# harshad16/odh-kubeflow

Measured on AMD Instinct MI355X. Metric: Notebook-CR reconciles/sec + p50 pod-Ready latency at 1/2/4/8 GPU pods, higher is better.
Workload: dtype n/a

## Files before the change

odh_kubeflow_amd/native/objcore.cpp:

```cpp
#define PY_SSIZE_T_CLEAN
#include <Python.h>

#include <cerrno>
#include <cmath>
#include <cstdio>
#include <cstdlib>
#include <cstring>
#include <string>
#include <string_view>
#include <unordered_map>
#include <utility>
#include <vector>

namespace {

PyObject* copy_tree(PyObject* o, int depth) {
  if (depth > 512) {
    PyErr_SetString(PyExc_RecursionError, "object tree too deep");
    return nullptr;
  }
  if (PyDict_CheckExact(o)) {
    PyObject* out = _PyDict_NewPresized(PyDict_GET_SIZE(o));
    if (!out) return nullptr;
    Py_ssize_t pos = 0;
    PyObject *k, *v;
    while (PyDict_Next(o, &pos, &k, &v)) {
      PyObject* c = copy_tree(v, depth + 1);
// ... 742 lines not shown
PyObject* py_loads_shared(PyObject*, PyObject* args) {
  PyObject *data, *old = Py_None;
  if (!PyArg_ParseTuple(args, "O|O", &data, &old)) return nullptr;
  Parser ps;
  if (!init_parser(data, &ps)) return nullptr;
  PyObject* out = value(ps, old == Py_None ? nullptr : old, 0);
  if (!out) return nullptr;
  ws(ps);
  if (ps.p != ps.end) {
    Py_DECREF(out);
    return fail(ps, "extra data");
  }
  return out;
}

PyObject* py_loads_event(PyObject*, PyObject* args) {
  PyObject *data, *lookup = Py_None;
  if (!PyArg_ParseTuple(args, "O|O", &data, &lookup)) return nullptr;
  Parser ps;
  if (!init_parser(data, &ps)) return nullptr;
  ws(ps);
  if (ps.p >= ps.end || *ps.p != '{') return fail(ps, "an event is an object");
  ++ps.p;
  PyObject* type = nullptr;
  PyObject* obj = nullptr;
  PyObject* ret = nullptr;
  ws(ps);
  if (ps.p < ps.end && *ps.p == '}') {
    ++ps.p;
  } else {
    while (true) {
      ws(ps);
      if (ps.p >= ps.end || *ps.p != '"') {
        fail(ps, "expected a key");
        goto done;
// ... 53 lines not shown
  }
  ws(ps);
  if (ps.p != ps.end) {
    fail(ps, "extra data");
    goto done;
  }
  if (!obj) obj = PyDict_New();
  if (!obj) goto done;
  ret = PyTuple_Pack(2, type ? type : Py_None, obj);
done:
  Py_XDECREF(type);
  Py_XDECREF(obj);
  return ret;
}


bool enc_value(std::string& out, PyObject* o, int depth);

void enc_string(std::string& out, PyObject* u) {
  Py_ssize_t n;
  const char* s = PyUnicode_AsUTF8AndSize(u, &n);
  out.push_back('"');
  const char* run = s;
  for (Py_ssize_t i = 0; i < n; ++i) {
    unsigned char c = static_cast<unsigned char>(s[i]);
    if (c >= 0x20 && c != '"' && c != '\\') continue;
    out.append(run, static_cast<size_t>(s + i - run));
    run = s + i + 1;
    switch (c) {
      case '"': out.append("\\\""); break;
// ... 100 lines not shown
  }
  PyErr_SetString(PyExc_TypeError, "not a JSON tree");
  return false;
}

PyObject* py_dumps(PyObject*, PyObject* o) {
  std::string out;
  out.reserve(1024);
  if (!enc_value(out, o, 0)) {
    if (!PyErr_Occurred()) PyErr_SetString(PyExc_TypeError, "not a JSON tree");
    return nullptr;
  }
  return PyBytes_FromStringAndSize(out.data(), static_cast<Py_ssize_t>(out.size()));
}

PyMethodDef methods[] = {
    {"dumps", py_dumps, METH_O,
     "dumps(obj) -> bytes: compact JSON (json.dumps with separators=(',', ':'), UTF-8) of a JSON tree."},
    {"deepcopy", py_deepcopy, METH_O, "Deep copy of a JSON tree (dict/list; tuples become lists)."},
    {"semantic_equal", py_semantic_equal, METH_VARARGS,
     "Structural equality treating missing/None/{}/[] map values as equal."},
    {"equal_except", py_equal_except, METH_VARARGS, "a == b ignoring the given metadata keys."},
    {"loads_shared", py_loads_shared, METH_VARARGS,
     "loads_shared(data, old=None): json.loads, reusing the subtrees of old the document leaves unchanged."},
    {"loads_event", py_loads_event, METH_VARARGS,
     "loads_event(line, lookup=None) -> (type, object): a watch event, the object decoded against "
     "lookup(namespace, name)."},
    {nullptr, nullptr, 0, nullptr}};

PyModuleDef module = {PyModuleDef_HEAD_INIT, "_objcore", "Native JSON-tree core", -1, methods,
                      nullptr, nullptr, nullptr, nullptr};

}

PyMODINIT_FUNC PyInit__objcore(void) {
  if (!g_keys) g_keys = new std::unordered_map<std::string_view, PyObject*>();
  return PyModule_Create(&module);
}
```

odh_kubeflow_amd/ops/build.py:

```python

from __future__ import annotations

import os
import shutil
import subprocess
import sys
import sysconfig
from typing import Dict, List

HERE = os.path.dirname(os.path.abspath(__file__))
CSRC = os.path.join(HERE, "csrc")
LIBDIR = os.path.join(HERE, "_lib")
NATIVE = os.path.join(os.path.dirname(HERE), "native")
TEST_NATIVE = os.path.join(os.path.dirname(HERE), "testing", "native")
OBJCORE = "_objcore" + (sysconfig.get_config_var("EXT_SUFFIX") or ".so")
ARCH = os.environ.get("ODH_GPU_ARCH", "gfx950")
ROCM = os.environ.get("ROCM_PATH", "/opt/rocm")
PROBE_EXE = "odh-gpu-probe"


def _hipcc() -> str:
    p = os.path.join(ROCM, "bin", "hipcc")
    return p if os.path.exists(p) else (shutil.which("hipcc") or p)

# ... 3 lines not shown
        "libodh_gpu_probe.so": {
            "src": [os.path.join(CSRC, "gpu_probe.hip"), os.path.join(CSRC, "probe_cli.cpp")],
            "deps": [os.path.join(CSRC, "gpu_probe.h"), os.path.join(CSRC, "gpu_probe_mx.h"),
                     os.path.join(CSRC, "gpu_probe_dense.h")],
            "cmd": lambda src, out: [_hipcc(), f"--offload-arch={ARCH}", "-O3", "-std=c++17", "-shared", "-fPIC",
                                     *src, "-o", out],
        },
        PROBE_EXE: {
            "src": [os.path.join(CSRC, "probe_main.cpp")],
            "deps": [os.path.join(LIBDIR, "libodh_gpu_probe.so")],
            "cmd": lambda src, out: [_hipcc(), "-O2", "-std=c++17", *src, f"-L{LIBDIR}", "-lodh_gpu_probe",
                                     "-Wl,-rpath,$ORIGIN", "-o", out],
        },
        OBJCORE: {
            "src": [os.path.join(NATIVE, "objcore.cpp")],
            "out": os.path.join(NATIVE, OBJCORE),
            "cmd": lambda src, out: [os.environ.get("CXX", "g++"), "-O2", "-std=c++17", "-shared", "-fPIC", "-Wall",
                                     "-fno-strict-aliasing", f"-I{sysconfig.get_paths()['include']}", *src,
                                     "-o", out],
        },
        "odh-apiserver": {
            "src": [os.path.join(TEST_NATIVE, "apiserver", "apiserver.cpp")],
            "deps": [os.path.join(TEST_NATIVE, "apiserver", "json.hpp")],
            "out": os.path.join(TEST_NATIVE, "bin", "odh-apiserver"),
            "cmd": lambda src, out: [os.environ.get("CXX", "g++"), "-O2", "-std=c++17", "-pthread", "-Wall", *src,
                                     "-o", out, "-lssl", "-lcrypto"],
        },
        "libodh_gpu_telemetry.so": {
            "src": [os.path.join(CSRC, "gpu_telemetry.cpp")],
            "cmd": lambda src, out: [os.environ.get("CXX", "g++"), "-O2", "-std=c++17", "-shared", "-fPIC",
# ... 47 lines not shown
```

odh_kubeflow_amd/runtime/http1.py:

```python

from __future__ import annotations

import asyncio
import os
import ssl as _ssl
import sys
import time
from typing import AsyncIterator, Dict, List, Optional, Tuple
from urllib.parse import urlsplit


class HttpError(Exception):
    pass


def _parse_head(raw: bytes) -> Tuple[int, Dict[str, str]]:
    lines = raw.decode("latin-1").split("\r\n")
    parts = lines[0].split(" ", 2)
    if len(parts) < 2 or not parts[0].startswith("HTTP/"):
        raise HttpError(f"bad status line {lines[0]!r}")
    headers = {}
    for line in lines[1:]:
        if ":" in line:
            k, v = line.split(":", 1)
# ... 41 lines not shown
    _LAG_LOOPS.add(id(loop))

    async def watch() -> None:
        while True:
            t0 = time.perf_counter()
            await asyncio.sleep(0.002)
            late = (time.perf_counter() - t0 - 0.002) * 1e3
            if late >= _STALL_MS:
                _stall_report(f"event loop {late:.1f} ms late")

    loop.create_task(watch())


class _Conn(asyncio.Protocol):

    def __init__(self):
        self.transport = None
        self.buf = bytearray()
        self.closed = False
        self._waiter: Optional[asyncio.Future] = None
        self._head: Optional[Tuple[int, Dict[str, str]]] = None
        self._body = bytearray()
        self._want = -1
        self._streaming = False
        self._lines: List[bytes] = []
        self._got = 0
        self._eof = False
        self._no_body = False


    def connection_made(self, transport) -> None:
        self.transport = transport

    def data_received(self, data: bytes) -> None:
        self.buf += data
        if self._waiter is not None or self._streaming:
            self._advance()

    def eof_received(self):
        return False

    def connection_lost(self, exc) -> None:
        self.closed = True
        self._eof = True
        w, self._waiter = self._waiter, None
        if w is None or w.done():
            return
        if self._streaming:
            w.set_result(None)
        elif self._want == -3 and self._head is not None:
            self._body += self.buf
            self.buf.clear()
            w.set_result((self._head[0], bytes(self._body), True))
        else:
            w.set_exception(ConnectionResetError(f"connection lost mid-response: {exc!r}"))


    def _advance(self) -> None:
        w = self._waiter
        try:
            if self._head is None:
                i = self.buf.find(b"\r\n\r\n")
                if i < 0:
                    return
                self._head = _parse_head(bytes(self.buf[:i]))
                del self.buf[:i + 4]
                status, h = self._head
                if self._no_body or status < 200 or status in (204, 304):
                    self._want = 0
                elif h.get("transfer-encoding", "").lower() == "chunked":
# ... 54 lines not shown
            del body[:start]
        if done:
            self._eof = True
            self.close()
        w = self._waiter
        if (self._lines or self._eof) and w is not None and not w.done():
            self._waiter = None
            w.set_result(None)


    async def roundtrip(self, payload: bytes) -> Tuple[int, bytes, bool]:
        if self.closed:
            raise ConnectionResetError("connection closed")
        self._waiter = w = asyncio.get_running_loop().create_future()
        self._no_body = payload.startswith(b"HEAD ")
        self.transport.write(payload)
        if self.buf:
            self._advance()
        return await w

    async def open_stream(self, payload: bytes) -> Tuple[int, Dict[str, str]]:
        if self.closed:
            raise ConnectionResetError("connection closed")
        self._streaming = True
        self._waiter = w = asyncio.get_running_loop().create_future()
        self.transport.write(payload)
        got = await w
        if got is None:
            raise ConnectionResetError("connection lost before the response head")
        return got

    async def next_lines(self) -> List[bytes]:
        while not self._lines:
            if self._eof or self.closed:
                return []
            self._waiter = w = asyncio.get_running_loop().create_future()
            try:
                await w
            finally:
                if self._waiter is w:
                    self._waiter = None
        out, self._lines = self._lines, []
        return out

    def close(self) -> None:
        self.closed = True
        if self.transport is not None:
            self.transport.close()


class Http1Pool:
    def __init__(self, base_url: str, ssl_context: Optional[_ssl.SSLContext] = None,
                 headers: Optional[Dict[str, str]] = None, size: int = 64, spare: int = 0):
        u = urlsplit(base_url)
        self.host = u.hostname or "127.0.0.1"
        self.port = u.port or (443 if u.scheme == "https" else 80)
        self.ssl = ssl_context if u.scheme == "https" else None
        self._hdr = {"Host": f"{self.host}:{self.port}", "Accept": "application/json"}
        self._hdr.update(headers or {})
        self._static = "".join(f"{k}: {v}\r\n" for k, v in self._hdr.items())
        self._idle: List[_Conn] = []
        self.size = size
        self.opened = 0
        self.spare = max(0, int(spare))
        self._warming = 0

    def set_header(self, name: str, value: Optional[str]) -> None:
        if value is None:
            self._hdr.pop(name, None)
        else:
            self._hdr[name] = value
        self._static = "".join(f"{k}: {v}\r\n" for k, v in self._hdr.items())

    async def _connect(self) -> _Conn:
        loop = asyncio.get_running_loop()
        transport, conn = await loop.create_connection(_Conn, self.host, self.port, ssl=self.ssl)
        sock = transport.get_extra_info("socket")
        if sock is not None:
            import socket

            try:
                sock.setsockopt(socket.IPPROTO_TCP, socket.TCP_NODELAY, 1)
            except OSError:
                pass
        self.opened += 1
        return conn

    def _head(self, method: str, target: str, body: Optional[bytes], content_type: Optional[str]) -> bytes:
        h = f"{method} {target} HTTP/1.1\r\n{self._static}"
        if body is not None:
            h += f"Content-Type: {content_type or 'application/json'}\r\nContent-Length: {len(body)}\r\n"
# ... 66 lines not shown
            raise
        return status, headers, _Stream(conn)

    async def close(self) -> None:
        self.spare = 0
        for c in self._idle:
            c.close()
        self._idle.clear()


class _Stream:

    def __init__(self, conn: _Conn):
        self.conn = conn

    async def read_all(self) -> bytes:
        try:
            out = []
            while True:
                got = await self.conn.next_lines()
                if not got:
                    break
                out += [x + b"\n" for x in got]
            return b"".join(out) + bytes(self.conn._body)
        finally:
            self.close()

    async def batches(self) -> AsyncIterator[List[bytes]]:
        try:
            while True:
                got = await self.conn.next_lines()
                if not got:
                    return
                yield got
        finally:
            self.close()

    async def lines(self) -> AsyncIterator[bytes]:
        async for batch in self.batches():
            for line in batch:
                yield line

    def close(self) -> None:
        self.conn.close()



_REASONS = {200: "OK", 400: "Bad Request", 404: "Not Found", 405: "Method Not Allowed", 413: "Payload Too Large",
            500: "Internal Server Error"}
Handler = "Callable[[str, str, Dict[str, str], bytes], Awaitable[Tuple[int, str, bytes]]]"


class Http1Server:

    def __init__(self, handler, host: str = "127.0.0.1", port: int = 0,
                 ssl_context: Optional[_ssl.SSLContext] = None, max_body: int = 16 << 20, reuse_port: bool = False,
                 max_requests_per_conn: int = 0):
        self.handler = handler
        self.reuse_port = reuse_port
        self.max_requests_per_conn = max_requests_per_conn
        self.host = host
        self.port = port
        self.ssl = ssl_context
        self.max_body = max_body
        self._server = None
        self._conns: set = set()

    async def start(self) -> "Http1Server":
        if _STALL_MS:
            _ensure_loop_watchdog()
        self._server = await asyncio.start_server(self._serve, self.host, self.port, ssl=self.ssl, limit=1 << 24,
                                                  reuse_port=self.reuse_port or None)
        self.port = self._server.sockets[0].getsockname()[1]
        return self

    async def _serve(self, reader, writer) -> None:
        task = asyncio.current_task()
        self._conns.add(task)
        sock = writer.get_extra_info("socket")
        if sock is not None:
            import socket

            try:
                sock.setsockopt(socket.IPPROTO_TCP, socket.TCP_NODELAY, 1)
            except OSError:
                pass
        served = 0
        try:
            while True:
                try:
                    raw = await reader.readuntil(b"\r\n\r\n")
                except (asyncio.IncompleteReadError, ConnectionError, OSError, _ssl.SSLError):
                    return
                lines = raw.decode("latin-1").split("\r\n")
                parts = lines[0].split(" ")
                if len(parts) < 3:
                    return
                method, target = parts[0], parts[1]
                headers = {}
                for line in lines[1:]:
                    if ":" in line:
                        k, v = line.split(":", 1)
                        headers[k.strip().lower()] = v.strip()
                n = int(headers.get("content-length", "0") or 0)
                if n > self.max_body:
                    status, ctype, body = 413, "text/plain", b"request body too large"
                else:
                    data = await reader.readexactly(n) if n else b""
                    try:
                        status, ctype, body = await self.handler(method, target.split("?", 1)[0], headers, data)
                    except Exception as e:
                        status, ctype, body = 500, "text/plain", repr(e).encode()
                served += 1
                close = headers.get("connection", "").lower() == "close" or (
                    self.max_requests_per_conn > 0 and served >= self.max_requests_per_conn)
                head = (f"HTTP/1.1 {status} {_REASONS.get(status, 'OK')}\r\nContent-Type: {ctype}\r\n"
                        f"Content-Length: {len(body)}\r\n{'Connection: close' + chr(13) + chr(10) if close else ''}\r\n")
                writer.write(head.encode("latin-1") + body)
                await writer.drain()
                if close:
                    return
        except (ConnectionError, OSError, asyncio.IncompleteReadError):
            return
        finally:
            self._conns.discard(task)
            try:
                writer.close()
            except Exception:
                pass

    async def stop(self) -> None:
        if self._server is not None:
            self._server.close()
            for t in list(self._conns):
                t.cancel()
            try:
                await asyncio.wait_for(self._server.wait_closed(), 2.0)
            except (asyncio.TimeoutError, Exception):
                pass
            self._server = None
```

odh_kubeflow_amd/runtime/rest.py:

```python

from __future__ import annotations

import asyncio
import base64
import json
import logging
import os
import ssl
import tempfile
import time
from dataclasses import dataclass, field
from typing import Any, AsyncIterator, Dict, List, Optional, Tuple

try:
    from ..native._objcore import dumps as _dumps
    from ..native._objcore import loads_event as _loads_event
    from ..native._objcore import loads_shared as _loads_shared

    def loads_json(raw):
        try:
            return _loads_shared(raw)
        except ValueError:
            return json.loads(raw)

# ... 165 lines not shown
            self.t = now
            if self.tokens >= 1:
                self.tokens -= 1
                return
            await asyncio.sleep((1 - self.tokens) / self.qps)


def _info_and_version(ref) -> Tuple[ResourceInfo, str]:
    info = SCHEME.resolve(ref)
    return info, _version_of(ref) or info.storage_version


class RestClient(Client):
    GET_RETRIES = 10

    def __init__(self, config: RestConfig, pool: int = 64):
        self.config = config
        self.base = config.host.rstrip("/")
        self._ssl = config.ssl_context()
        self._session = None
        self._pool = pool
        self._bucket = TokenBucket(config.qps, config.burst)
        self.requests = 0
        self.by_verb: Dict[str, int] = {}
        self.bytes_in: Dict[str, int] = {}
        from collections import deque

        self.get_ms = deque(maxlen=8192)
        self.retries = 0
        self.user = config.user_agent
        self._discovery: dict = {}
        self.tokens: Optional[FileTokenSource] = (FileTokenSource(config.token_file, config.token)
                                                  if config.token_file else None)
        self._sent_token: Optional[str] = None
        self.token_retries = 0

    def _bearer(self) -> Optional[str]:
        return self.tokens.token() if self.tokens is not None else self.config.token

    def _http(self):
        from .http1 import Http1Pool

        tok = self._bearer()
        if self._session is None:
            headers = {"User-Agent": self.config.user_agent}
            if tok:
                headers["Authorization"] = f"Bearer {tok}"
            self._session = Http1Pool(self.base, self._ssl, headers, size=self._pool, spare=2)
            self._sent_token = tok
        elif tok != self._sent_token:
            self._session.set_header("Authorization", f"Bearer {tok}" if tok else None)
            self._sent_token = tok
        return self._session

    def _unauthorized_retry(self, status: int, sent: Optional[str]) -> bool:
        if status != 401 or self.tokens is None:
            return False
        self.tokens.refresh()
        if self.tokens.token() == sent:
            return False
        self.token_retries += 1
        return True

# ... 190 lines not shown
            if self._unauthorized_retry(status, sent):
                status, _headers, stream = await self._http().stream("GET", target)
            else:
                status, _headers, stream = 401, _headers, None
        if stream is None:
            raise ApiError.from_status({"code": 401, "reason": "Unauthorized", "message": "Unauthorized"}, 401)
        if status >= 400:
            raw = await stream.read_all()
            try:
                raise ApiError.from_status(json.loads(raw), status)
            except ValueError:
                raise InternalError(raw[:200].decode(errors="replace"))
        loads = json.loads
        native = _loads_event
        try:
            async for lines in stream.batches():
                out = []
                err = None
                for line in lines:
                    if not line or line.isspace():
                        continue
                    if native is not None:
                        try:
                            et, obj = native(line, lookup)
                        except ValueError:
                            ev = loads(line)
                            et, obj = ev.get("type"), ev.get("object") or {}
                    else:
                        ev = loads(line)
                        et, obj = ev.get("type"), ev.get("object") or {}
# ... 13 lines not shown
```

Before: 3396.

## Move HTTP/1.1 framing and watch-stream decoding into native C++ parser

Adds a C++ wire framer (wire.hpp) exposed as ResponseParser, WatchDecoder and RequestParser types in _objcore. The client pool, the test server and the watch loop use them to frame responses, de-chunk watch bodies, split lines and decode events in one native call, replacing per-line Python work. The server switches from asyncio streams to a Protocol backed by the native request parser. The aim is lower Python overhead per request and per watch event, at the cost of a large new native parsing surface with its own edge cases and error handling.

```diff
diff --git a/odh_kubeflow_amd/native/objcore.cpp b/odh_kubeflow_amd/native/objcore.cpp
--- a/odh_kubeflow_amd/native/objcore.cpp
+++ b/odh_kubeflow_amd/native/objcore.cpp
@@ -6,11 +6,14 @@
 #include <cstdio>
 #include <cstdlib>
 #include <cstring>
+#include <new>
 #include <string>
 #include <string_view>
 #include <unordered_map>
 #include <utility>
 #include <vector>
+
+#include "wire.hpp"
 
 namespace {
 
@@ -783,11 +786,7 @@
   return out;
 }
 
-PyObject* py_loads_event(PyObject*, PyObject* args) {
-  PyObject *data, *lookup = Py_None;
-  if (!PyArg_ParseTuple(args, "O|O", &data, &lookup)) return nullptr;
-  Parser ps;
-  if (!init_parser(data, &ps)) return nullptr;
+PyObject* decode_event(Parser& ps, PyObject* lookup) {
   ws(ps);
   if (ps.p >= ps.end || *ps.p != '{') return fail(ps, "an event is an object");
   ++ps.p;
@@ -871,6 +870,14 @@
   return ret;
 }
 
+PyObject* py_loads_event(PyObject*, PyObject* args) {
+  PyObject *data, *lookup = Py_None;
+  if (!PyArg_ParseTuple(args, "O|O", &data, &lookup)) return nullptr;
+  Parser ps;
+  if (!init_parser(data, &ps)) return nullptr;
+  return decode_event(ps, lookup);
+}
+
 
 bool enc_value(std::string& out, PyObject* o, int depth);
 
@@ -1001,6 +1008,364 @@
   return PyBytes_FromStringAndSize(out.data(), static_cast<Py_ssize_t>(out.size()));
 }
 
+
+PyObject* wire_error(const std::string& what) {
+  PyErr_Format(PyExc_ValueError, "malformed HTTP message: %s", what.empty() ? "?" : what.c_str());
+  return nullptr;
+}
+
+inline PyObject* view_bytes(wire::View v) {
+  return PyBytes_FromStringAndSize(v.p, static_cast<Py_ssize_t>(v.n));
+}
+
+inline PyObject* view_latin1(wire::View v) {
+  return PyUnicode_DecodeLatin1(v.p ? v.p : "", static_cast<Py_ssize_t>(v.n), nullptr);
+}
+
+bool append_owned(PyObject* list, PyObject* item) {
+  if (!item) return false;
+  int rc = PyList_Append(list, item);
+  Py_DECREF(item);
+  return rc == 0;
+}
+
+struct ResponseParserObj {
+  PyObject_HEAD
+  wire::ResponseFramer* f;
+};
+
+PyObject* rp_new(PyTypeObject* t, PyObject*, PyObject*) {
+  auto* self = reinterpret_cast<ResponseParserObj*>(t->tp_alloc(t, 0));
+  if (!self) return nullptr;
+  self->f = new (std::nothrow) wire::ResponseFramer();
+  if (!self->f) {
+    Py_DECREF(self);
+    return PyErr_NoMemory();
+  }
+  return reinterpret_cast<PyObject*>(self);
+}
+
+void rp_dealloc(PyObject* o) {
+  delete reinterpret_cast<ResponseParserObj*>(o)->f;
+  Py_TYPE(o)->tp_free(o);
+}
+
+PyObject* response_tuple(const wire::Response& r) {
+  PyObject* body = view_bytes(r.body);
+  if (!body) return nullptr;
+  PyObject* t = Py_BuildValue("(iNO)", r.status, body, r.close ? Py_True : Py_False);
+  return t;
+}
+
+PyObject* rp_feed(PyObject* o, PyObject* arg) {
+  auto* self = reinterpret_cast<ResponseParserObj*>(o);
+  Py_buffer b;
+  if (PyObject_GetBuffer(arg, &b, PyBUF_SIMPLE) < 0) return nullptr;
+  PyObject* out = PyList_New(0);
+  const char* p = static_cast<const char*>(b.buf);
+  size_t n = static_cast<size_t>(b.len);
+  try {
+    while (out) {
+      size_t used = 0;
+      wire::Response r;
+      wire::Result got = self->f->next(p, n, &used, &r);
+      if (got == wire::kError) {
+        Py_CLEAR(out);
+        wire_error(self->f->error());
+        break;
+      }
+      if (got == wire::kNeedMore) break;
+      if (!append_owned(out, response_tuple(r))) Py_CLEAR(out);
+      p += used;
+      n -= used;
+      if (n == 0 && !self->f->mid_response()) break;
+    }
+  } catch (...) {
+    Py_CLEAR(out);
+    PyErr_NoMemory();
+  }
+  PyBuffer_Release(&b);
+  return out;
+}
+
+PyObject* rp_finish(PyObject* o, PyObject*) {
+  auto* self = reinterpret_cast<ResponseParserObj*>(o);
+  wire::Response r;
+  if (self->f->finish(&r) == wire::kReady) return response_tuple(r);
+  Py_RETURN_NONE;
+}
+
+PyObject* rp_set_head(PyObject* o, PyObject* arg) {
+  int v = PyObject_IsTrue(arg);
+  if (v < 0) return nullptr;
+  reinterpret_cast<ResponseParserObj*>(o)->f->set_head_request(v != 0);
+  Py_RETURN_NONE;
+}
+
+PyObject* rp_feed_head(PyObject* o, PyObject* arg) {
+  auto* self = reinterpret_cast<ResponseParserObj*>(o);
+  Py_buffer b;
+  if (PyObject_GetBuffer(arg, &b, PyBUF_SIMPLE) < 0) return nullptr;
+  PyObject* out = nullptr;
+  try {
+    size_t used = 0;
+    wire::ResponseHead h;
+    wire::BodyMode mode;
+    uint64_t length;
+    wire::Result got = self->f->head(static_cast<const char*>(b.buf), static_cast<size_t>(b.len), &used, &h, &mode,
+                                     &length);
+    if (got == wire::kError) {
+      wire_error(self->f->error());
+    } else if (got == wire::kNeedMore) {
+      out = Py_None;
+      Py_INCREF(out);
+    } else {
+      out = Py_BuildValue("(iOiKy#)", h.status, h.close ? Py_True : Py_False, static_cast<int>(mode),
+                          static_cast<unsigned long long>(length), static_cast<const char*>(b.buf) + used,
+                          static_cast<Py_ssize_t>(static_cast<size_t>(b.len) - used));
+    }
+  } catch (...) {
+    PyErr_NoMemory();
+  }
+  PyBuffer_Release(&b);
+  return out;
+}
+
+PyMethodDef rp_methods[] = {
+    {"feed", rp_feed, METH_O, "feed(data) -> [(status, body, close), ...]"},
+    {"finish", rp_finish, METH_NOARGS, "finish() -> (status, body, True) or None: the connection ended"},
+    {"set_head", rp_set_head, METH_O, "set_head(flag): the next response answers a HEAD"},
+    {"feed_head", rp_feed_head, METH_O, "feed_head(data) -> None or (status, close, mode, length, rest)"},
+    {nullptr, nullptr, 0, nullptr}};
+
+PyTypeObject ResponseParserType{};
+
+struct WatchDecoderObj {
+  PyObject_HEAD
+  wire::StreamFramer* f;
+  bool busy;
+};
+
+PyObject* wd_new(PyTypeObject* t, PyObject* args, PyObject*) {
+  int mode = wire::kChunked;
+  unsigned long long length = 0;
+  if (!PyArg_ParseTuple(args, "|iK", &mode, &length)) return nullptr;
+  if (mode < wire::kLength || mode > wire::kUntilEof) {
+    PyErr_SetString(PyExc_ValueError, "mode is 0 (length), 1 (chunked) or 2 (until EOF)");
+    return nullptr;
+  }
+  auto* self = reinterpret_cast<WatchDecoderObj*>(t->tp_alloc(t, 0));
+  if (!self) return nullptr;
+  self->busy = false;
+  self->f = new (std::nothrow) wire::StreamFramer(static_cast<wire::BodyMode>(mode), length);
+  if (!self->f) {
+    Py_DECREF(self);
+    return PyErr_NoMemory();
+  }
+  return reinterpret_cast<PyObject*>(self);
+}
+
+void wd_dealloc(PyObject* o) {
+  delete reinterpret_cast<WatchDecoderObj*>(o)->f;
+  Py_TYPE(o)->tp_free(o);
+}
+
+inline bool blank_line(const char* p, size_t n) {
+  for (size_t i = 0; i < n; ++i) {
+    char c = p[i];
+    if (!(c == ' ' || (c >= '\t' && c <= '\r'))) return false;
+  }
+  return true;
+}
+
+PyObject* wd_run(WatchDecoderObj* self, PyObject* data, PyObject* lookup, bool decode) {
+  if (self->busy) {
+    PyErr_SetString(PyExc_RuntimeError, "WatchDecoder.feed re-entered from its lookup");
+    return nullptr;
+  }
+  Py_buffer b;
+  if (PyObject_GetBuffer(data, &b, PyBUF_SIMPLE) < 0) return nullptr;
+  PyObject* out = PyList_New(0);
+  bool ok = out != nullptr;
+  wire::Result got = wire::kNeedMore;
+  self->busy = true;
+  try {
+    Parser ps;
+    auto line = [&](const char* p, size_t n) {
+      if (!ok) return;
+      if (!decode) {
+        ok = append_owned(out, PyBytes_FromStringAndSize(p, static_cast<Py_ssize_t>(n)));
+        return;
+      }
+      if (blank_line(p, n)) return;
+      ps.p = p;
+      ps.end = p + n;
+      PyObject* ev = decode_event(ps, lookup);
+      if (!ev && PyErr_ExceptionMatches(PyExc_ValueError)) {
+        PyErr_Clear();
+        ev = PyBytes_FromStringAndSize(p, static_cast<Py_ssize_t>(n));
+      }
+      ok = append_owned(out, ev);
+    };
+    if (ok) got = self->f->feed(static_cast<const char*>(b.buf), static_cast<size_t>(b.len), line);
+  } catch (...) {
+    if (ok) PyErr_NoMemory();
+    ok = false;
+  }
+  self->busy = false;
+  PyBuffer_Release(&b);
+  if (ok && got == wire::kError) {
+    ok = false;
+    wire_error("bad chunk");
+  }
+  if (!ok) {
+    Py_XDECREF(out);
+    return nullptr;
+  }
+  return Py_BuildValue("(NO)", out, got == wire::kReady ? Py_True : Py_False);
+}
+
+PyObject* wd_feed(PyObject* o, PyObject* args) {
+  PyObject *data, *lookup = Py_None;
+  if (!PyArg_ParseTuple(args, "O|O", &data, &lookup)) return nullptr;
+  return wd_run(reinterpret_cast<WatchDecoderObj*>(o), data, lookup, true);
+}
+
+PyObject* wd_feed_lines(PyObject* o, PyObject* data) {
+  return wd_run(reinterpret_cast<WatchDecoderObj*>(o), data, Py_None, false);
+}
+
+PyObject* wd_rest(PyObject* o, PyObject*) {
+  const std::string& r = reinterpret_cast<WatchDecoderObj*>(o)->f->rest();
+  return PyBytes_FromStringAndSize(r.data(), static_cast<Py_ssize_t>(r.size()));
+}
+
+PyObject* wd_done(PyObject* o, PyObject*) {
+  return PyBool_FromLong(reinterpret_cast<WatchDecoderObj*>(o)->f->done());
+}
+
+PyMethodDef wd_methods[] = {
+    {"feed", wd_feed, METH_VARARGS, "feed(data, lookup=None) -> (events, done)"},
+    {"feed_lines", wd_feed_lines, METH_O, "feed_lines(data) -> (lines, done)"},
+    {"rest", wd_rest, METH_NOARGS, "rest() -> bytes after the last newline"},
+    {"done", wd_done, METH_NOARGS, "done() -> the body has ended"},
+    {nullptr, nullptr, 0, nullptr}};
+
+PyTypeObject WatchDecoderType{};
+
+struct RequestParserObj {
+  PyObject_HEAD
+  wire::RequestFramer* f;
+};
+
+PyObject* rq_new(PyTypeObject* t, PyObject* args, PyObject*) {
+  unsigned long long max_body = 16ull << 20;
+  if (!PyArg_ParseTuple(args, "|K", &max_body)) return nullptr;
+  auto* self = reinterpret_cast<RequestParserObj*>(t->tp_alloc(t, 0));
+  if (!self) return nullptr;
+  self->f = new (std::nothrow) wire::RequestFramer(max_body);
+  if (!self->f) {
+    Py_DECREF(self);
+    return PyErr_NoMemory();
+  }
+  return reinterpret_cast<PyObject*>(self);
+}
+
+void rq_dealloc(PyObject* o) {
+  delete reinterpret_cast<RequestParserObj*>(o)->f;
+  Py_TYPE(o)->tp_free(o);
+}
+
+PyObject* request_tuple(const wire::Request& r) {
+  PyObject* headers = PyDict_New();
+  if (!headers) return nullptr;
+  for (const auto& kv : r.headers) {
+    PyObject* k = view_latin1(kv.first);
+    PyObject* v = view_latin1(kv.second);
+    int rc = (k && v) ? PyDict_SetItem(headers, k, v) : -1;
+    Py_XDECREF(k);
+    Py_XDECREF(v);
+    if (rc < 0) {
+      Py_DECREF(headers);
+      return nullptr;
+    }
+  }
+  PyObject* body;
+  if (r.too_large) {
+    body = Py_None;
+    Py_INCREF(body);
+  } else {
+    body = view_bytes(r.body);
+  }
+  PyObject* method = view_latin1(r.method);
+  PyObject* path = view_latin1(r.path);
+  if (!body || !method || !path) {
+    Py_XDECREF(body);
+    Py_XDECREF(method);
+    Py_XDECREF(path);
+    Py_DECREF(headers);
+    return nullptr;
+  }
+  return Py_BuildValue("(NNNN)", method, path, headers, body);
+}
+
+PyObject* rq_feed(PyObject* o, PyObject* arg) {
+  auto* self = reinterpret_cast<RequestParserObj*>(o);
+  Py_buffer b;
+  if (PyObject_GetBuffer(arg, &b, PyBUF_SIMPLE) < 0) return nullptr;
+  PyObject* out = PyList_New(0);
+  const char* p = static_cast<const char*>(b.buf);
+  size_t n = static_cast<size_t>(b.len);
+  try {
+    wire::Request r;
+    while (out) {
+      size_t used = 0;
+      wire::Result got = self->f->next(p, n, &used, &r);
+      if (got == wire::kError) {
+        Py_CLEAR(out);
+        wire_error(self->f->error());
+        break;
+      }
+      if (got == wire::kNeedMore) break;
+      if (!append_owned(out, request_tuple(r))) Py_CLEAR(out);
+      p += used;
+      n -= used;
+      if (n == 0) break;
+    }
+  } catch (...) {
+    Py_CLEAR(out);
+    PyErr_NoMemory();
+  }
+  PyBuffer_Release(&b);
+  return out;
+}
+
+PyMethodDef rq_methods[] = {
+    {"feed", rq_feed, METH_O, "feed(data) -> [(method, path, headers, body), ...]"},
+    {nullptr, nullptr, 0, nullptr}};
+
+PyTypeObject RequestParserType{};
+
+bool add_type(PyObject* m, PyTypeObject* t, const char* name, const char* qualname, size_t size, newfunc nw,
+              destructor de, PyMethodDef* meths, const char* doc) {
+  PyObject* as_object = reinterpret_cast<PyObject*>(t);
+  if (Py_REFCNT(as_object) == 0) Py_SET_REFCNT(as_object, 1);
+  t->tp_name = qualname;
+  t->tp_basicsize = static_cast<Py_ssize_t>(size);
+  t->tp_flags = Py_TPFLAGS_DEFAULT;
+  t->tp_new = nw;
+  t->tp_dealloc = de;
+  t->tp_methods = meths;
+  t->tp_doc = doc;
+  if (PyType_Ready(t) < 0) return false;
+  Py_INCREF(t);
+  if (PyModule_AddObject(m, name, reinterpret_cast<PyObject*>(t)) < 0) {
+    Py_DECREF(t);
+    return false;
+  }
+  return true;
+}
+
 PyMethodDef methods[] = {
     {"dumps", py_dumps, METH_O,
      "dumps(obj) -> bytes: compact JSON (json.dumps with separators=(',', ':'), UTF-8) of a JSON tree."},
@@ -1022,5 +1387,17 @@
 
 PyMODINIT_FUNC PyInit__objcore(void) {
   if (!g_keys) g_keys = new std::unordered_map<std::string_view, PyObject*>();
-  return PyModule_Create(&module);
-}
+  PyObject* m = PyModule_Create(&module);
+  if (!m) return nullptr;
+  if (!add_type(m, &ResponseParserType, "ResponseParser", "_objcore.ResponseParser", sizeof(ResponseParserObj), rp_new,
+                rp_dealloc, rp_methods, "Incremental HTTP/1.1 response framing (client side).") ||
+      !add_type(m, &WatchDecoderType, "WatchDecoder", "_objcore.WatchDecoder", sizeof(WatchDecoderObj), wd_new,
+                wd_dealloc, wd_methods,
+                "WatchDecoder(mode=1, length=0): a streaming body framed, split into lines and decoded.") ||
+      !add_type(m, &RequestParserType, "RequestParser", "_objcore.RequestParser", sizeof(RequestParserObj), rq_new,
+                rq_dealloc, rq_methods, "RequestParser(max_body=16 MiB): incremental HTTP/1.1 request framing.")) {
+    Py_DECREF(m);
+    return nullptr;
+  }
+  return m;
+}
diff --git a/odh_kubeflow_amd/native/wire.hpp b/odh_kubeflow_amd/native/wire.hpp
--- /dev/null
+++ b/odh_kubeflow_amd/native/wire.hpp
@@ -0,0 +1,570 @@
+#pragma once
+
+#include <cstddef>
+#include <cstdint>
+#include <cstring>
+#include <string>
+#include <utility>
+#include <vector>
+
+namespace wire {
+
+enum Result { kNeedMore = 0, kReady = 1, kError = -1 };
+enum BodyMode { kLength = 0, kChunked = 1, kUntilEof = 2 };
+
+constexpr size_t kMaxHead = 1 << 20;
+constexpr int kMaxDigits = 12;
+
+struct View {
+  const char* p = nullptr;
+  size_t n = 0;
+};
+
+inline bool is_lws(char c) { return c == ' ' || c == '\t'; }
+
+inline View trim(const char* p, size_t n) {
+  while (n && is_lws(*p)) ++p, --n;
+  while (n && is_lws(p[n - 1])) --n;
+  return {p, n};
+}
+
+inline char lower(char c) { return (c >= 'A' && c <= 'Z') ? static_cast<char>(c + 32) : c; }
+
+inline bool ieq(View v, const char* word) {
+  size_t n = std::strlen(word);
+  if (v.n != n) return false;
+  for (size_t i = 0; i < n; ++i)
+    if (lower(v.p[i]) != word[i]) return false;
+  return true;
+}
+
+inline bool parse_dec(View v, uint64_t* out) {
+  if (v.n == 0 || v.n > static_cast<size_t>(kMaxDigits)) return false;
+  uint64_t x = 0;
+  for (size_t i = 0; i < v.n; ++i) {
+    if (v.p[i] < '0' || v.p[i] > '9') return false;
+    x = x * 10 + static_cast<uint64_t>(v.p[i] - '0');
+  }
+  *out = x;
+  return true;
+}
+
+inline bool parse_hex(View v, uint64_t* out) {
+  if (v.n == 0 || v.n > static_cast<size_t>(kMaxDigits)) return false;
+  uint64_t x = 0;
+  for (size_t i = 0; i < v.n; ++i) {
+    char c = v.p[i];
+    int d;
+    if (c >= '0' && c <= '9') d = c - '0';
+    else if (c >= 'a' && c <= 'f') d = c - 'a' + 10;
+    else if (c >= 'A' && c <= 'F') d = c - 'A' + 10;
+    else return false;
+    x = (x << 4) | static_cast<uint64_t>(d);
+  }
+  *out = x;
+  return true;
+}
+
+inline size_t find_seq(const char* p, size_t n, size_t from, const char* pat, size_t m) {
+  while (from + m <= n) {
+    const void* q = std::memchr(p + from, pat[0], n - from - (m - 1));
+    if (!q) return n;
+    size_t i = static_cast<size_t>(static_cast<const char*>(q) - p);
+    if (std::memcmp(p + i, pat, m) == 0) return i;
+    from = i + 1;
+  }
+  return n;
+}
+
+class Until {
+ public:
+  Result take(const char* p, size_t n, const char* term, size_t m, size_t* used, View* out) {
+    if (held_) {
+      buf_.clear();
+      held_ = false;
+    }
+    if (buf_.empty()) {
+      size_t i = find_seq(p, n, 0, term, m);
+      if (i < n) {
+        *out = {p, i};
+        *used = i + m;
+        return kReady;
+      }
+      if (n > kMaxHead) return kError;
+      buf_.assign(p, n);
+      *used = n;
+      return kNeedMore;
+    }
+    size_t old = buf_.size();
+    size_t from = old >= m - 1 ? old - (m - 1) : 0;
+    size_t head = n < m - 1 ? n : m - 1;
+    buf_.append(p, head);
+    size_t i = find_seq(buf_.data(), buf_.size(), from, term, m);
+    if (i < buf_.size()) {
+      *used = i + m - old;
+      buf_.resize(i);
+      *out = {buf_.data(), buf_.size()};
+      held_ = true;
+      return kReady;
+    }
+    size_t j = find_seq(p, n, 0, term, m);
+    if (j < n) {
+      buf_.resize(old);
+      buf_.append(p, j);
+      *used = j + m;
+      *out = {buf_.data(), buf_.size()};
+      held_ = true;
+      return kReady;
+    }
+    buf_.append(p + head, n - head);
+    *used = n;
+    if (buf_.size() > kMaxHead) return kError;
+    return kNeedMore;
+  }
+  void reset() {
+    buf_.clear();
+    held_ = false;
+  }
+
+ private:
+  std::string buf_;
+  bool held_ = false;
+};
+
+template <class F>
+inline void each_header(View block, F&& f) {
+  size_t pos = find_seq(block.p, block.n, 0, "\r\n", 2);
+  while (pos < block.n) {
+    pos += 2;
+    size_t e = find_seq(block.p, block.n, pos, "\r\n", 2);
+    const char* line = block.p + pos;
+    size_t ln = e - pos;
+    const void* c = ln ? std::memchr(line, ':', ln) : nullptr;
+    if (c) {
+      size_t k = static_cast<size_t>(static_cast<const char*>(c) - line);
+      f(trim(line, k), trim(line + k + 1, ln - k - 1));
+    }
+    pos = e;
+  }
+}
+
+inline View first_line(View block) {
+  return {block.p, find_seq(block.p, block.n, 0, "\r\n", 2)};
+}
+
+class Dechunker {
+ public:
+  template <class F>
+  Result feed(const char* p, size_t n, size_t* used, F&& data) {
+    size_t i = 0;
+    while (true) {
+      if (state_ == kData) {
+        if (i >= n) break;
+        size_t k = n - i < left_ ? n - i : static_cast<size_t>(left_);
+        data(p + i, k);
+        i += k;
+        left_ -= k;
+        if (left_ == 0) {
+          state_ = kDataEnd;
+          left_ = 2;
+        }
+        continue;
+      }
+      if (state_ == kDataEnd) {
+        if (i >= n) break;
+        if (p[i] != (left_ == 2 ? '\r' : '\n')) return kError;
+        ++i;
+        if (--left_ == 0) state_ = kSize;
+        continue;
+      }
+      if (i >= n) break;
+      size_t u = 0;
+      View line;
+      Result r = line_.take(p + i, n - i, "\r\n", 2, &u, &line);
+      i += u;
+      if (r == kError) return kError;
+      if (r == kNeedMore) break;
+      if (state_ == kSize) {
+        const void* semi = line.n ? std::memchr(line.p, ';', line.n) : nullptr;
+        size_t k = semi ? static_cast<size_t>(static_cast<const char*>(semi) - line.p) : line.n;
+        uint64_t size;
+        if (!parse_hex(trim(line.p, k), &size)) return kError;
+        if (size == 0) {
+          state_ = kTrailer;
+        } else {
+          state_ = kData;
+          left_ = size;
+        }
+      } else {
+        if (line.n == 0) {
+          state_ = kSize;
+          *used = i;
+          return kReady;
+        }
+      }
+    }
+    *used = n;
+    return kNeedMore;
+  }
+  void reset() {
+    state_ = kSize;
+    left_ = 0;
+    line_.reset();
+  }
+
+ private:
+  enum State { kSize, kData, kDataEnd, kTrailer };
+  State state_ = kSize;
+  uint64_t left_ = 0;
+  Until line_;
+};
+
+struct Response {
+  int status = 0;
+  bool close = false;
+  View body;
+};
+
+struct ResponseHead {
+  int status = 0;
+  bool close = false;
+  bool has_length = false;
+  bool chunked = false;
+  uint64_t length = 0;
+};
+
+inline bool parse_response_head(View block, ResponseHead* h, std::string* err) {
+  View sl = first_line(block);
+  if (sl.n < 5 || std::memcmp(sl.p, "HTTP/", 5) != 0) {
+    *err = "bad status line";
+    return false;
+  }
+  const void* sp = std::memchr(sl.p, ' ', sl.n);
+  if (!sp) {
+    *err = "bad status line";
+    return false;
+  }
+  const char* s = static_cast<const char*>(sp) + 1;
+  size_t rest = static_cast<size_t>(sl.p + sl.n - s);
+  const void* sp2 = rest ? std::memchr(s, ' ', rest) : nullptr;
+  size_t sn = sp2 ? static_cast<size_t>(static_cast<const char*>(sp2) - s) : rest;
+  uint64_t code;
+  if (!parse_dec({s, sn}, &code) || code > 999) {
+    *err = "bad status code";
+    return false;
+  }
+  *h = ResponseHead();
+  h->status = static_cast<int>(code);
+  bool ok = true;
+  each_header(block, [&](View k, View v) {
+    if (ieq(k, "content-length")) {
+      h->has_length = true;
+      if (!parse_dec(v, &h->length)) ok = false;
+    } else if (ieq(k, "transfer-encoding")) {
+      h->chunked = ieq(v, "chunked");
+    } else if (ieq(k, "connection")) {
+      h->close = ieq(v, "close");
+    }
+  });
+  if (!ok) *err = "bad content-length";
+  return ok;
+}
+
+inline void body_rule(const ResponseHead& h, bool head_request, bool streaming, BodyMode* mode, uint64_t* length) {
+  *length = 0;
+  if (head_request || h.status < 200 || h.status == 204 || h.status == 304) {
+    *mode = kLength;
+  } else if (h.chunked) {
+    *mode = kChunked;
+  } else if (h.has_length) {
+    *mode = kLength;
+    *length = h.length;
+  } else if (h.close || streaming) {
+    *mode = kUntilEof;
+  } else {
+    *mode = kLength;
+  }
+}
+
+class ResponseFramer {
+ public:
+  void set_head_request(bool v) { head_request_ = v; }
+
+  Result next(const char* p, size_t n, size_t* used, Response* r) {
+    *used = 0;
+    if (failed_) return kError;
+    size_t i = 0;
+    if (state_ == kHead) {
+      size_t u = 0;
+      View block;
+      Result got = head_.take(p, n, "\r\n\r\n", 4, &u, &block);
+      i = u;
+      *used = i;
+      if (got == kError) return fail("header block too long");
+      if (got == kNeedMore) return kNeedMore;
+      if (!parse_response_head(block, &h_, &err_)) return fail(nullptr);
+      body_rule(h_, head_request_, false, &mode_, &left_);
+      body_.clear();
+      state_ = kBody;
+      if (mode_ == kLength && left_ <= n - i) {
+        *r = {h_.status, h_.close, {p + i, static_cast<size_t>(left_)}};
+        *used = i + static_cast<size_t>(left_);
+        state_ = kHead;
+        return kReady;
+      }
+      if (mode_ == kChunked) chunks_.reset();
+    }
+    if (mode_ == kLength) {
+      size_t k = n - i < left_ ? n - i : static_cast<size_t>(left_);
+      body_.append(p + i, k);
+      left_ -= k;
+      *used = i + k;
+      if (left_) return kNeedMore;
+    } else if (mode_ == kChunked) {
+      size_t u = 0;
+      Result got = chunks_.feed(p + i, n - i, &u, [&](const char* d, size_t k) { body_.append(d, k); });
+      *used = i + u;
+      if (got == kError) return fail("bad chunk");
+      if (got == kNeedMore) return kNeedMore;
+    } else {
+      body_.append(p + i, n - i);
+      *used = n;
+      return kNeedMore;
+    }
+    *r = {h_.status, h_.close, {body_.data(), body_.size()}};
+    state_ = kHead;
+    return kReady;
+  }
+
+  Result finish(Response* r) {
+    if (failed_) return kError;
+    if (state_ == kBody && mode_ == kUntilEof) {
+      *r = {h_.status, true, {body_.data(), body_.size()}};
+      state_ = kHead;
+      return kReady;
+    }
+    if (state_ == kBody) return fail("connection ended mid-response");
+    return kNeedMore;
+  }
+
+  Result head(const char* p, size_t n, size_t* used, ResponseHead* h, BodyMode* mode, uint64_t* length) {
+    *used = 0;
+    if (failed_) return kError;
+    View block;
+    Result got = head_.take(p, n, "\r\n\r\n", 4, used, &block);
+    if (got == kError) return fail("header block too long");
+    if (got == kNeedMore) return kNeedMore;
+    if (!parse_response_head(block, h, &err_)) return fail(nullptr);
+    body_rule(*h, head_request_, true, mode, length);
+    return kReady;
+  }
+
+  bool mid_response() const { return state_ == kBody; }
+  const std::string& error() const { return err_; }
+
+ private:
+  Result fail(const char* what) {
+    if (what) err_ = what;
+    failed_ = true;
+    return kError;
+  }
+  enum State { kHead, kBody };
+  State state_ = kHead;
+  bool head_request_ = false;
+  bool failed_ = false;
+  ResponseHead h_;
+  BodyMode mode_ = kLength;
+  uint64_t left_ = 0;
+  Until head_;
+  Dechunker chunks_;
+  std::string body_;
+  std::string err_;
+};
+
+class StreamFramer {
+ public:
+  StreamFramer(BodyMode mode, uint64_t length) : mode_(mode), left_(length) {
+    done_ = mode == kLength && length == 0;
+  }
+
+  template <class F>
+  Result feed(const char* p, size_t n, F&& line) {
+    if (failed_) return kError;
+    if (done_) return kReady;
+    auto data = [&](const char* d, size_t k) { split(d, k, line); };
+    if (mode_ == kChunked) {
+      size_t used = 0;
+      Result got = chunks_.feed(p, n, &used, data);
+      if (got == kError) {
+        failed_ = true;
+        return kError;
+      }
+      done_ = got == kReady;
+    } else if (mode_ == kLength) {
+      size_t k = n < left_ ? n : static_cast<size_t>(left_);
+      data(p, k);
+      left_ -= k;
+      done_ = left_ == 0;
+    } else {
+      data(p, n);
+    }
+    return done_ ? kReady : kNeedMore;
+  }
+
+  bool done() const { return done_; }
+  const std::string& rest() const { return partial_; }
+
+ private:
+  template <class F>
+  void split(const char* d, size_t k, F&& line) {
+    while (k) {
+      const void* q = std::memchr(d, '\n', k);
+      if (!q) {
+        partial_.append(d, k);
+        return;
+      }
+      size_t i = static_cast<size_t>(static_cast<const char*>(q) - d);
+      if (partial_.empty()) {
+        line(d, i);
+      } else {
+        partial_.append(d, i);
+        line(partial_.data(), partial_.size());
+        partial_.clear();
+      }
+      d += i + 1;
+      k -= i + 1;
+    }
+  }
+  BodyMode mode_;
+  uint64_t left_;
+  bool done_ = false;
+  bool failed_ = false;
+  Dechunker chunks_;
+  std::string partial_;
+};
+
+struct Request {
+  View method;
+  View target;
+  View path;
+  bool close = false;
+  bool too_large = false;
+  std::vector<std::pair<View, View>> headers;
+  View body;
+};
+
+class RequestFramer {
+ public:
+  explicit RequestFramer(uint64_t max_body) : max_body_(max_body) {}
+
+  Result next(const char* p, size_t n, size_t* used, Request* r) {
+    *used = 0;
+    if (failed_) return kError;
+    size_t i = 0;
+    if (state_ == kSkip) {
+      size_t k = n < left_ ? n : static_cast<size_t>(left_);
+      left_ -= k;
+      i = k;
+      *used = i;
+      if (left_) return kNeedMore;
+      state_ = kHead;
+    }
+    if (state_ == kHead) {
+      if (i >= n) return kNeedMore;
+      size_t u = 0;
+      View block;
+      Result got = until_.take(p + i, n - i, "\r\n\r\n", 4, &u, &block);
+      i += u;
+      *used = i;
+      if (got == kError) return fail("header block too long");
+      if (got == kNeedMore) return kNeedMore;
+      head_.assign(block.p, block.n);
+      if (!parse_head()) return fail("bad request line");
+      body_.clear();
+      if (length_ > max_body_) {
+        state_ = length_ ? kSkip : kHead;
+        left_ = length_;
+        fill(r, {nullptr, 0});
+        r->too_large = true;
+        return kReady;
+      }
+      left_ = length_;
+      if (left_ <= n - i) {
+        fill(r, {p + i, static_cast<size_t>(left_)});
+        *used = i + static_cast<size_t>(left_);
+        return kReady;
+      }
+      state_ = kBody;
+    }
+    size_t k = n - i < left_ ? n - i : static_cast<size_t>(left_);
+    body_.append(p + i, k);
+    left_ -= k;
+    *used = i + k;
+    if (left_) return kNeedMore;
+    state_ = kHead;
+    fill(r, {body_.data(), body_.size()});
+    return kReady;
+  }
+
+  const std::string& error() const { return err_; }
+
+ private:
+  Result fail(const char* what) {
+    err_ = what;
+    failed_ = true;
+    return kError;
+  }
+  bool parse_head() {
+    View block{head_.data(), head_.size()};
+    View rl = first_line(block);
+    const void* a = rl.n ? std::memchr(rl.p, ' ', rl.n) : nullptr;
+    if (!a) return false;
+    const char* t = static_cast<const char*>(a) + 1;
+    size_t rest = static_cast<size_t>(rl.p + rl.n - t);
+    const void* b = rest ? std::memchr(t, ' ', rest) : nullptr;
+    if (!b) return false;
+    method_ = {rl.p, static_cast<size_t>(static_cast<const char*>(a) - rl.p)};
+    target_ = {t, static_cast<size_t>(static_cast<const char*>(b) - t)};
+    headers_.clear();
+    length_ = 0;
+    close_ = false;
+    bool ok = true;
+    char* base = &head_[0];
+    each_header(block, [&](View k, View v) {
+      for (size_t j = 0; j < k.n; ++j) base[k.p - base + j] = lower(k.p[j]);
+      headers_.emplace_back(k, v);
+      if (ieq(k, "content-length")) {
+        if (v.n == 0) length_ = 0;
+        else if (!parse_dec(v, &length_)) ok = false;
+      } else if (ieq(k, "connection")) {
+        close_ = ieq(v, "close");
+      }
+    });
+    return ok;
+  }
+  void fill(Request* r, View body) {
+    r->method = method_;
+    r->target = target_;
+    const void* q = target_.n ? std::memchr(target_.p, '?', target_.n) : nullptr;
+    r->path = {target_.p, q ? static_cast<size_t>(static_cast<const char*>(q) - target_.p) : target_.n};
+    r->close = close_;
+    r->too_large = false;
+    r->headers = headers_;
+    r->body = body;
+  }
+  enum State { kHead, kBody, kSkip };
+  State state_ = kHead;
+  bool failed_ = false;
+  uint64_t max_body_;
+  uint64_t length_ = 0;
+  uint64_t left_ = 0;
+  bool close_ = false;
+  View method_, target_;
+  std::vector<std::pair<View, View>> headers_;
+  Until until_;
+  std::string head_;
+  std::string body_;
+  std::string err_;
+};
+
+}
diff --git a/odh_kubeflow_amd/ops/build.py b/odh_kubeflow_amd/ops/build.py
--- a/odh_kubeflow_amd/ops/build.py
+++ b/odh_kubeflow_amd/ops/build.py
@@ -41,6 +41,7 @@
         },
         OBJCORE: {
             "src": [os.path.join(NATIVE, "objcore.cpp")],
+            "deps": [os.path.join(NATIVE, "wire.hpp")],
             "out": os.path.join(NATIVE, OBJCORE),
             "cmd": lambda src, out: [os.environ.get("CXX", "g++"), "-O2", "-std=c++17", "-shared", "-fPIC", "-Wall",
                                      "-fno-strict-aliasing", f"-I{sysconfig.get_paths()['include']}", *src,
diff --git a/odh_kubeflow_amd/runtime/http1.py b/odh_kubeflow_amd/runtime/http1.py
--- a/odh_kubeflow_amd/runtime/http1.py
+++ b/odh_kubeflow_amd/runtime/http1.py
@@ -8,6 +8,23 @@
 import time
 from typing import AsyncIterator, Dict, List, Optional, Tuple
 from urllib.parse import urlsplit
+
+try:
+    from ..native._objcore import RequestParser as _RequestParser
+    from ..native._objcore import ResponseParser as _ResponseParser
+    from ..native._objcore import WatchDecoder as _WatchDecoder
+except ImportError:
+    _RequestParser = _ResponseParser = _WatchDecoder = None
+
+NATIVE_WIRE = _ResponseParser is not None and os.environ.get("ODH_WIRE", "").strip().lower() != "python"
+
+
+def _use_native(native: Optional[bool]) -> bool:
+    if native is None:
+        return NATIVE_WIRE
+    if native and _ResponseParser is None:
+        raise RuntimeError("the native framing needs _objcore (python -m odh_kubeflow_amd.ops.build)")
+    return bool(native)
 
 
 class HttpError(Exception):
@@ -79,7 +96,13 @@
 
 class _Conn(asyncio.Protocol):
 
-    def __init__(self):
+    def __init__(self, native: Optional[bool] = None):
+        self.native = _use_native(native)
+        self._parser = _ResponseParser() if self.native else None
+        self._pending: List[bytes] = []
+        self._ready: list = []
+        self._arrivals: List[bytes] = []
+        self._decoder = None
         self.transport = None
         self.buf = bytearray()
         self.closed = False
@@ -98,6 +121,21 @@
         self.transport = transport
 
     def data_received(self, data: bytes) -> None:
+        if self.native:
+            if self._decoder is not None:
+                self._arrivals.append(data)
+                w = self._waiter
+                if w is not None:
+                    self._waiter = None
+                    if not w.done():
+                        w.set_result(None)
+            elif self._waiter is None:
+                self._pending.append(data)
+            elif self._streaming:
+                self._feed_head(data)
+            else:
+                self._feed(data)
+            return
         self.buf += data
         if self._waiter is not None or self._streaming:
             self._advance()
@@ -113,12 +151,71 @@
             return
         if self._streaming:
             w.set_result(None)
+        elif self.native:
+            got = self._parser.finish()
+            if got is not None:
+                w.set_result(got)
+            else:
+                w.set_exception(ConnectionResetError(f"connection lost mid-response: {exc!r}"))
         elif self._want == -3 and self._head is not None:
             self._body += self.buf
             self.buf.clear()
             w.set_result((self._head[0], bytes(self._body), True))
         else:
             w.set_exception(ConnectionResetError(f"connection lost mid-response: {exc!r}"))
+
+
+    def _fail(self, w, e: Exception) -> None:
+        self._waiter = None
+        self.close()
+        if w is not None and not w.done():
+            w.set_exception(HttpError(f"bad response: {e!r}"))
+
+    def _feed(self, data: bytes) -> None:
+        w = self._waiter
+        try:
+            got = self._parser.feed(data)
+        except ValueError as e:
+            self._fail(w, e)
+            return
+        if got:
+            self._waiter = None
+            if len(got) > 1:
+                self._ready += got[1:]
+            if not w.done():
+                w.set_result(got[0])
+
+    def _feed_head(self, data: bytes) -> None:
+        w = self._waiter
+        try:
+            got = self._parser.feed_head(data)
+        except ValueError as e:
+            self._fail(w, e)
+            return
+        if got is None:
+            return
+        status, close, mode, length, rest = got
+        self._decoder = _WatchDecoder(mode, length)
+        if rest:
+            self._arrivals.append(rest)
+        if self._decoder.done():
+            self._eof = True
+        self._waiter = None
+        if not w.done():
+            w.set_result((status, {"connection": "close"} if close else {}))
+
+    async def next_arrivals(self) -> List[bytes]:
+        while not self._arrivals:
+            if self._eof or self.closed:
+                return []
+            self._waiter = w = asyncio.get_running_loop().create_future()
+            try:
+                await w
+            finally:
+                if self._waiter is w:
+                    self._waiter = None
+        out, self._arrivals = self._arrivals, []
+        return out
 
 
     def _advance(self) -> None:
@@ -203,6 +300,17 @@
             raise ConnectionResetError("connection closed")
         self._waiter = w = asyncio.get_running_loop().create_future()
         self._no_body = payload.startswith(b"HEAD ")
+        if self.native:
+            self._parser.set_head(self._no_body)
+            self.transport.write(payload)
+            if self._ready:
+                self._waiter = None
+                w.set_result(self._ready.pop(0))
+            elif self._pending:
+                data = b"".join(self._pending)
+                self._pending.clear()
+                self._feed(data)
+            return await w
         self.transport.write(payload)
         if self.buf:
             self._advance()
@@ -214,6 +322,10 @@
         self._streaming = True
         self._waiter = w = asyncio.get_running_loop().create_future()
         self.transport.write(payload)
+        if self.native and self._pending:
+            data = b"".join(self._pending)
+            self._pending.clear()
+            self._feed_head(data)
         got = await w
         if got is None:
             raise ConnectionResetError("connection lost before the response head")
@@ -240,7 +352,9 @@
 
 class Http1Pool:
     def __init__(self, base_url: str, ssl_context: Optional[_ssl.SSLContext] = None,
-                 headers: Optional[Dict[str, str]] = None, size: int = 64, spare: int = 0):
+                 headers: Optional[Dict[str, str]] = None, size: int = 64, spare: int = 0,
+                 native: Optional[bool] = None):
+        self.native = _use_native(native)
         u = urlsplit(base_url)
         self.host = u.hostname or "127.0.0.1"
         self.port = u.port or (443 if u.scheme == "https" else 80)
@@ -263,7 +377,7 @@
 
     async def _connect(self) -> _Conn:
         loop = asyncio.get_running_loop()
-        transport, conn = await loop.create_connection(_Conn, self.host, self.port, ssl=self.ssl)
+        transport, conn = await loop.create_connection(lambda: _Conn(self.native), self.host, self.port, ssl=self.ssl)
         sock = transport.get_extra_info("socket")
         if sock is not None:
             import socket
@@ -360,7 +474,48 @@
     def __init__(self, conn: _Conn):
         self.conn = conn
 
+    async def _framed(self, lookup, decode: bool):
+        conn = self.conn
+        dec = conn._decoder
+        feed = dec.feed if decode else dec.feed_lines
+        try:
+            while True:
+                got = conn._arrivals
+                if got:
+                    conn._arrivals = []
+                else:
+                    got = await conn.next_arrivals()
+                    if not got:
+                        return
+                try:
+                    if len(got) == 1:
+                        out, done = feed(got[0], lookup) if decode else feed(got[0])
+                    else:
+                        out, done = [], False
+                        for data in got:
+                            part, done = feed(data, lookup) if decode else feed(data)
+                            out += part
+                            if done:
+                                break
+                except ValueError as e:
+                    raise HttpError(f"bad response: {e!r}") from e
+                if done:
+                    conn._eof = True
+                    conn.close()
+                if out:
+                    yield out
+        finally:
+            conn.close()
+
+    def event_batches(self, lookup=None) -> AsyncIterator[list]:
+        return self._framed(lookup, True)
+
     async def read_all(self) -> bytes:
+        if self.conn.native:
+            out = []
+            async for lines in self._framed(None, False):
+                out += [x + b"\n" for x in lines]
+            return b"".join(out) + self.conn._decoder.rest()
         try:
             out = []
             while True:
@@ -372,7 +527,10 @@
         finally:
             self.close()
 
-    async def batches(self) -> AsyncIterator[List[bytes]]:
+    def batches(self) -> AsyncIterator[List[bytes]]:
+        return self._framed(None, False) if self.conn.native else self._py_batches()
+
+    async def _py_batches(self) -> AsyncIterator[List[bytes]]:
         try:
             while True:
                 got = await self.conn.next_lines()
@@ -397,11 +555,149 @@
 Handler = "Callable[[str, str, Dict[str, str], bytes], Awaitable[Tuple[int, str, bytes]]]"
 
 
+class _PyRequestParser:
+
+    def __init__(self, max_body: int = 16 << 20):
+        self.max_body = max_body
+        self.buf = bytearray()
+        self._head: Optional[Tuple[str, str, Dict[str, str]]] = None
+        self._want = 0
+        self._skip = 0
+
+    def feed(self, data: bytes) -> List[Tuple[str, str, Dict[str, str], Optional[bytes]]]:
+        buf = self.buf
+        buf += data
+        out = []
+        while True:
+            if self._skip:
+                n = min(self._skip, len(buf))
+                del buf[:n]
+                self._skip -= n
+                if self._skip:
+                    break
+            if self._head is None:
+                i = buf.find(b"\r\n\r\n")
+                if i < 0:
+                    break
+                lines = bytes(buf[:i]).decode("latin-1").split("\r\n")
+                del buf[:i + 4]
+                parts = lines[0].split(" ")
+                if len(parts) < 3:
+                    raise ValueError(f"bad request line {lines[0]!r}")
+                headers = {}
+                for line in lines[1:]:
+                    if ":" in line:
+                        k, v = line.split(":", 1)
+                        headers[k.strip(" \t").lower()] = v.strip(" \t")
+                length = headers.get("content-length", "")
+                if length and not (length.isdigit() and length.isascii() and len(length) <= 12):
+                    raise ValueError(f"bad content-length {length!r}")
+                self._want = int(length or 0)
+                self._head = (parts[0], parts[1].split("?", 1)[0], headers)
+                if self._want > self.max_body:
+                    out.append((*self._head, None))
+                    self._head, self._skip = None, self._want
+                    continue
+            if len(buf) < self._want:
+                break
+            body = bytes(buf[:self._want])
+            del buf[:self._want]
+            out.append((*self._head, body))
+            self._head = None
+        return out
+
+
+class _ServerConn(asyncio.Protocol):
+
+    def __init__(self, server: "Http1Server"):
+        self.server = server
+        self.parser = _RequestParser(server.max_body) if server.native else _PyRequestParser(server.max_body)
+        self.transport = None
+        self.served = 0
+        self.queue: list = []
+        self.task: Optional[asyncio.Task] = None
+        self.closing = False
+
+    def connection_made(self, transport) -> None:
+        self.transport = transport
+        self.server._conns.add(self)
+        sock = transport.get_extra_info("socket")
+        if sock is not None:
+            import socket
+
+            try:
+                sock.setsockopt(socket.IPPROTO_TCP, socket.TCP_NODELAY, 1)
+            except OSError:
+                pass
+
+    def data_received(self, data: bytes) -> None:
+        if self.closing:
+            return
+        try:
+            got = self.parser.feed(data)
+        except ValueError:
+            self.abort()
+            return
+        if got:
+            self.queue += got
+            if self.task is None:
+                self._next()
+
+    def eof_received(self):
+        return False
+
+    def connection_lost(self, exc) -> None:
+        self.closing = True
+        self.server._conns.discard(self)
+        if self.task is not None:
+            self.task.cancel()
+
+    def abort(self) -> None:
+        self.closing = True
+        if self.task is not None:
+            self.task.cancel()
+        if self.transport is not None:
+            self.transport.close()
+
+    def _next(self) -> None:
+        while self.queue and not self.closing:
+            method, path, headers, body = self.queue.pop(0)
+            if body is None:
+                self._respond(headers, 413, "text/plain", b"request body too large")
+                continue
+            self.task = asyncio.get_running_loop().create_task(self._run(method, path, headers, body))
+            return
+
+    async def _run(self, method: str, path: str, headers: Dict[str, str], body: bytes) -> None:
+        try:
+            try:
+                status, ctype, out = await self.server.handler(method, path, headers, body)
+            except Exception as e:
+                status, ctype, out = 500, "text/plain", repr(e).encode()
+            if not self.closing:
+                self._respond(headers, status, ctype, out)
+        finally:
+            self.task = None
+        self._next()
+
+    def _respond(self, headers: Dict[str, str], status: int, ctype: str, body: bytes) -> None:
+        self.served += 1
+        limit = self.server.max_requests_per_conn
+        close = headers.get("connection", "").lower() == "close" or (limit > 0 and self.served >= limit)
+        head = (f"HTTP/1.1 {status} {_REASONS.get(status, 'OK')}\r\nContent-Type: {ctype}\r\n"
+                f"Content-Length: {len(body)}\r\n{'Connection: close' + chr(13) + chr(10) if close else ''}\r\n")
+        self.transport.write(head.encode("latin-1") + body)
+        if close:
+            self.closing = True
+            self.transport.close()
+
+
 class Http1Server:
 
     def __init__(self, handler, host: str = "127.0.0.1", port: int = 0,
                  ssl_context: Optional[_ssl.SSLContext] = None, max_body: int = 16 << 20, reuse_port: bool = False,
-                 max_requests_per_conn: int = 0):
+                 max_requests_per_conn: int = 0, native: Optional[bool] = None):
+        self.native = _use_native(native)
         self.handler = handler
         self.reuse_port = reuse_port
         self.max_requests_per_conn = max_requests_per_conn
@@ -415,71 +711,16 @@
     async def start(self) -> "Http1Server":
         if _STALL_MS:
             _ensure_loop_watchdog()
-        self._server = await asyncio.start_server(self._serve, self.host, self.port, ssl=self.ssl, limit=1 << 24,
-                                                  reuse_port=self.reuse_port or None)
+        self._server = await asyncio.get_running_loop().create_server(
+            lambda: _ServerConn(self), self.host, self.port, ssl=self.ssl, reuse_port=self.reuse_port or None)
         self.port = self._server.sockets[0].getsockname()[1]
         return self
-
-    async def _serve(self, reader, writer) -> None:
-        task = asyncio.current_task()
-        self._conns.add(task)
-        sock = writer.get_extra_info("socket")
-        if sock is not None:
-            import socket
-
-            try:
-                sock.setsockopt(socket.IPPROTO_TCP, socket.TCP_NODELAY, 1)
-            except OSError:
-                pass
-        served = 0
-        try:
-            while True:
-                try:
-                    raw = await reader.readuntil(b"\r\n\r\n")
-                except (asyncio.IncompleteReadError, ConnectionError, OSError, _ssl.SSLError):
-                    return
-                lines = raw.decode("latin-1").split("\r\n")
-                parts = lines[0].split(" ")
-                if len(parts) < 3:
-                    return
-                method, target = parts[0], parts[1]
-                headers = {}
-                for line in lines[1:]:
-                    if ":" in line:
-                        k, v = line.split(":", 1)
-                        headers[k.strip().lower()] = v.strip()
-                n = int(headers.get("content-length", "0") or 0)
-                if n > self.max_body:
-                    status, ctype, body = 413, "text/plain", b"request body too large"
-                else:
-                    data = await reader.readexactly(n) if n else b""
-                    try:
-                        status, ctype, body = await self.handler(method, target.split("?", 1)[0], headers, data)
-                    except Exception as e:
-                        status, ctype, body = 500, "text/plain", repr(e).encode()
-                served += 1
-                close = headers.get("connection", "").lower() == "close" or (
-                    self.max_requests_per_conn > 0 and served >= self.max_requests_per_conn)
-                head = (f"HTTP/1.1 {status} {_REASONS.get(status, 'OK')}\r\nContent-Type: {ctype}\r\n"
-                        f"Content-Length: {len(body)}\r\n{'Connection: close' + chr(13) + chr(10) if close else ''}\r\n")
-                writer.write(head.encode("latin-1") + body)
-                await writer.drain()
-                if close:
-                    return
-        except (ConnectionError, OSError, asyncio.IncompleteReadError):
-            return
-        finally:
-            self._conns.discard(task)
-            try:
-                writer.close()
-            except Exception:
-                pass
 
     async def stop(self) -> None:
         if self._server is not None:
             self._server.close()
-            for t in list(self._conns):
-                t.cancel()
+            for c in list(self._conns):
+                c.abort()
             try:
                 await asyncio.wait_for(self._server.wait_closed(), 2.0)
             except (asyncio.TimeoutError, Exception):
diff --git a/odh_kubeflow_amd/runtime/rest.py b/odh_kubeflow_amd/runtime/rest.py
--- a/odh_kubeflow_amd/runtime/rest.py
+++ b/odh_kubeflow_amd/runtime/rest.py
@@ -203,8 +203,9 @@
 class RestClient(Client):
     GET_RETRIES = 10
 
-    def __init__(self, config: RestConfig, pool: int = 64):
+    def __init__(self, config: RestConfig, pool: int = 64, native_wire: Optional[bool] = None):
         self.config = config
+        self._native_wire = native_wire
         self.base = config.host.rstrip("/")
         self._ssl = config.ssl_context()
         self._session = None
@@ -235,7 +236,8 @@
             headers = {"User-Agent": self.config.user_agent}
             if tok:
                 headers["Authorization"] = f"Bearer {tok}"
-            self._session = Http1Pool(self.base, self._ssl, headers, size=self._pool, spare=2)
+            self._session = Http1Pool(self.base, self._ssl, headers, size=self._pool, spare=2,
+                                      native=self._native_wire)
             self._sent_token = tok
         elif tok != self._sent_token:
             self._session.set_header("Authorization", f"Bearer {tok}" if tok else None)
@@ -456,6 +458,24 @@
         loads = json.loads
         native = _loads_event
         try:
+            if stream.conn.native:
+                async for events in stream.event_batches(lookup):
+                    err = None
+                    for i, ev in enumerate(events):
+                        if ev.__class__ is bytes:
+                            ev = loads(ev)
+                            events[i] = ev = (ev.get("type"), ev.get("object") or {})
+                        if ev[0] == "ERROR":
+                            err = ApiError.from_status(ev[1])
+                            del events[i:]
+                            break
+                    if events:
+                        yield events
+                    if err is not None:
+                        if err.code == 410:
+                            raise Gone(err.message)
+                        raise err
+                return
             async for lines in stream.batches():
                 out = []
                 err = None
```

Result: faster. 3604, median of 6 (+6.1%).
